# IST-DASLab/torch_cgx

Hardware: AMD Instinct MI355X
Metric: DDP samples/sec ResNet-50 4-bit (higher is better)
Workload: dtype bf16; 1 GPU; model=resnet50, global_batch=256, input=3x224x224, parallelism=dp1, backend=cgx, bits=4, bucket_size=1024, compression_active=False

## Files before the change

csrc/bindings.cc:

```cpp
#include <torch/extension.h>

#include <ATen/hip/impl/HIPStreamMasqueradingAsCUDA.h>
#include <torch/csrc/utils/pybind.h>

#include <ATen/hip/impl/HIPGuardImplMasqueradingAsCUDA.h>

#include <cstring>
#include <functional>
#include <thread>
#include <tuple>

#include "backend.h"
#include "bn_plan.h"
#include "collectives.h"
#include "conv1x1_plan.h"
#include "reducer.h"

namespace cgx {
namespace {

void run_rank_threads(int ws, int dev,
                      const std::function<void(int, hipStream_t)>& body,
                      const std::function<void()>& abort) {
  std::vector<hipStream_t> qs(ws, nullptr);
// ... 908 lines not shown
  }
  return out;
}

at::Tensor py_conv1x1_walk(int64_t rows, int64_t k, int64_t n,
                           int64_t max_workgroups) {
  const Conv1x1Plan p = conv1x1_plan(rows, k, n, (int)max_workgroups);
  TORCH_CHECK(p.eligible, "conv1x1_walk: shape is not eligible");
  return conv1x1_walk_of(p);
}


int clamp_workgroups(int64_t max_workgroups) {
  return (int)std::min<int64_t>(max_workgroups, 1 << 20);
}

bool py_conv1x1_bwd_eligible(const at::Tensor& dy, const at::Tensor& weight,
                             const c10::optional<at::Tensor>& skip) {
  if (!(bn_tensor_ok(dy) && weight.is_cuda() &&
        weight.device() == dy.device() &&
        weight.scalar_type() == at::kBFloat16 && weight.dim() == 4 &&
        weight.size(0) == dy.size(1) && weight.size(2) == 1 &&
        weight.size(3) == 1 && weight.is_contiguous() &&
        reinterpret_cast<uintptr_t>(weight.data_ptr()) % 16 == 0 &&
        conv1x1_bwd_plan(dy.numel() / dy.size(1), weight.size(1),
                         weight.size(0), skip.has_value())
            .eligible))
    return false;
  if (!skip.has_value()) return true;
  const at::Tensor& s = *skip;
  return s.dim() == 4 && s.size(0) == dy.size(0) &&
         s.size(1) == weight.size(1) && s.size(2) == dy.size(2) &&
         s.size(3) == dy.size(3) && s.device() == dy.device() &&
         bn_tensor_ok(s);
}

at::Tensor py_conv1x1_bwd_data(const at::Tensor& dy, const at::Tensor& weight,
                               const c10::optional<at::Tensor>& skip,
                               int64_t max_workgroups) {
  TORCH_CHECK(max_workgroups >= 0, "conv1x1_bwd_data: max_workgroups >= 0");
  TORCH_CHECK(py_conv1x1_bwd_eligible(dy, weight, skip),
              "conv1x1_bwd_data: dy, weight or skip is not eligible");
  const Conv1x1Plan p = conv1x1_bwd_plan(
      dy.numel() / dy.size(1), weight.size(1), weight.size(0),
      skip.has_value(), clamp_workgroups(max_workgroups));
  c10::hip::HIPGuardMasqueradingAsCUDA guard(dy.device().index());
  auto dx = at::empty({dy.size(0), p.n, dy.size(2), dy.size(3)}, dy.options(),
                      at::MemoryFormat::ChannelsLast);
  launch_conv1x1_bwd_data(p, dy.data_ptr(), weight.data_ptr(),
                          skip.has_value() ? skip->data_ptr() : nullptr,
                          dx.data_ptr(), bn_stream(dy));
  return dx;
}

py::dict py_conv1x1_bwd_plan(int64_t rows, int64_t k, int64_t n, bool with_add,
                             int64_t max_workgroups) {
  const Conv1x1Plan p =
      conv1x1_bwd_plan(rows, k, n, with_add, clamp_workgroups(max_workgroups));
  py::dict d;
  d["eligible"] = p.eligible;
  d["native"] = p.native;
  d["threads"] = kConvThreads;
  d["tile_rows"] = kConvTileRows;
  d["mfma_tiles"] = p.nt;
  d["tile_channels"] = p.bn;
  d["ntiles"] = p.ntiles;
  d["k_chunk"] = p.kc;
  d["k_chunks"] = p.nchunks;
  d["resident"] = p.resident;
  d["row_tiles"] = p.row_tiles;
  d["splits"] = p.splits;
  d["grid"] = p.grid;
  d["tiles_per_split"] = p.tiles_per_split;
  d["lds_bytes"] = p.lds_bytes;
  return d;
}

at::Tensor py_conv1x1_bwd_walk(int64_t rows, int64_t k, int64_t n,
                               bool with_add, int64_t max_workgroups) {
  const Conv1x1Plan p =
      conv1x1_bwd_plan(rows, k, n, with_add, clamp_workgroups(max_workgroups));
  TORCH_CHECK(p.eligible, "conv1x1_bwd_walk: shape is not eligible");
  return conv1x1_walk_of(p);
}

void py_register_layer(int64_t bucket_idx, int64_t layer_idx, int64_t numel,
                       int64_t bits, int64_t bucket_size) {
  Registry::get().register_layer((int)bucket_idx, (int)layer_idx, numel,
                                 (int)bits, (int)bucket_size);
}

void py_set_bits(int64_t bucket_idx, int64_t layer_idx, int64_t bits) {
  Registry::get().set_bits((int)bucket_idx, (int)layer_idx, (int)bits);
}

void py_set_bucket(int64_t bucket_idx, int64_t layer_idx,
                   int64_t bucket_size) {
  Registry::get().set_bucket_size((int)bucket_idx, (int)layer_idx,
                                  (int)bucket_size);
}

}
}

PYBIND11_MODULE(TORCH_EXTENSION_NAME, m) {
  py::class_<cgx::ProcessGroupCGX,
             c10::intrusive_ptr<cgx::ProcessGroupCGX>, c10d::Backend>(
      m, "ProcessGroupCGX")
      .def(py::init<c10::intrusive_ptr<c10d::Store>, int, int,
                    c10::intrusive_ptr<c10d::Backend>>(),
           py::arg("store"), py::arg("rank"), py::arg("size"),
           py::arg("cpu_delegate") = nullptr);

  m.def("register_layer", &cgx::py_register_layer, py::arg("bucket_idx"),
        py::arg("layer_idx"), py::arg("layer_numel"), py::arg("bits"),
        py::arg("bucket_size"));
  m.def("set_quantization_bits", &cgx::py_set_bits);
  m.def("set_quantization_bucket_size", &cgx::py_set_bucket);
  m.def("clear_registry", [] { cgx::Registry::get().clear(); });
  m.def("registry_match",
        [](int64_t numel, int64_t key) {
          cgx::Registry::BucketInfo info;
          const bool ok = cgx::Registry::get().next(
              numel, reinterpret_cast<const void*>(key), &info);
          return py::make_tuple(ok, ok ? info.idx : -1);
        },
        py::arg("numel"), py::arg("key") = 0);
  m.def("registry_snapshot", [] {
    py::list out;
    auto& reg = cgx::Registry::get();
    for (const auto& b : reg.snapshot()) {
      py::list numels, cfgs;
      for (auto n : b.numels) numels.append(n);
      for (const auto& c : b.cfgs)
        cfgs.append(py::make_tuple(c.bits, c.bucket_size));
      out.append(py::make_tuple(b.idx, numels, cfgs));
    }
    return out;
  });

  m.def("parse_engine_config", [] {
    auto c = cgx::EngineConfig::from_env();
    py::dict d;
    d["fusion_bytes"] = c.fusion_bytes;
    d["min_elems"] = c.min_elems;
    d["default_bits"] = c.default_bits;
    d["default_bucket"] = c.default_bucket;
    d["stochastic"] = c.stochastic;
    d["inner_ring"] = c.ring;
    d["cross_ring"] = c.cross_ring;
    d["debug_a2a"] = c.debug_a2a;
    d["fake_ratio"] = c.fake_ratio;
    d["skip_incomplete"] = c.skip_incomplete;
    d["dummy"] = c.dummy;
    d["intra_compress"] = c.intra_compress;
    d["intra_broadcast"] = c.intra_broadcast;
    d["error_feedback"] = c.error_feedback;
    return d;
  });
  m.def("env_flag", &cgx::env_flag, py::arg("name"),
        py::arg("default") = false,
        "Test seam: the textual boolean parser (only \"0\" is false).");
  m.def("env_int", &cgx::env_int, py::arg("name"), py::arg("default"),
        "Test seam: the numeric parser behind the `!= 0` booleans.");
  m.def("loopback_allreduce", &cgx::py_loopback_allreduce, py::arg("buckets"),
        "Run Reducer::allreduce (flat) at world_size=len(buckets) on one GPU "
// ... 51 lines not shown
        py::arg("dummy") = false,
        "Test seam: the bucket plan for layers laid out back to back from "
        "byte offset 0 -> (uncomp [(byte_off, count)], chunks [[(byte_off, "
        "numel, bits, bucket)]]).");
  m.def("plan_chunk", &cgx::py_plan_chunk, py::arg("views"), py::arg("dtype"),
        py::arg("ws"), py::arg("skip_incomplete") = false,
        "Test seam: the rank plan of one chunk [(byte_off, numel, bits, "
        "bucket)] -> (offs, szs, comp, rs [[(byte_off, n, bits, bucket, "
        "comp_off, skip_incomplete, fb_off)]]).");
  m.def("route_quantize", &cgx::py_route_quantize, py::arg("slices"),
        "Test seam: the launch router's quantize plan for "
        "[(in, out, fb, n, bits, bucket, skip_incomplete)] (pointers as "
        "ints) -> [(bits, kind, descs, cum, any_residual, max_gpl)].");
  m.def("route_dequantize", &cgx::py_route_dequantize, py::arg("slices"),
        py::arg("dtype"), py::arg("src_stride") = 0, py::arg("nsrc") = 1,
        py::arg("add") = false,
        "Test seam: the launch router's dequantize plan for "
        "[(in, out, n, bits, bucket, skip_incomplete)] -> "
        "[(bits, kind, descs, total_groups, any_residual)].");
  m.def("bn_act_forward", &cgx::py_bn_act_forward, py::arg("x"),
        py::arg("identity"), py::arg("weight"), py::arg("bias"),
        py::arg("running_mean"), py::arg("running_var"), py::arg("momentum"),
        py::arg("eps"), py::arg("relu"), py::arg("part") = py::none(),
        "Training-mode BatchNorm2d of a channels_last bf16 tensor, fused with "
        "an optional residual add and ReLU -> (out, mean, invstd, mask | "
        "None); updates the running statistics in place.  With `part`, the "
        "partials conv1x1_stats returned with x, the statistics pass over x "
        "is skipped.");
  m.def("bn_act_backward", &cgx::py_bn_act_backward, py::arg("dy"),
        py::arg("x"), py::arg("mean"), py::arg("invstd"), py::arg("weight"),
        py::arg("mask"), py::arg("has_identity"),
        "Backward of bn_act_forward -> (dx, dgamma, dbeta, didentity | None).");
  m.def("bn_act2_forward", &cgx::py_bn_act2_forward, py::arg("x3"),
        py::arg("xd"), py::arg("weight3"), py::arg("bias3"),
        py::arg("running_mean3"), py::arg("running_var3"),
        py::arg("momentum3"), py::arg("eps3"), py::arg("weightd"),
        py::arg("biasd"), py::arg("running_meand"), py::arg("running_vard"),
        py::arg("momentumd"), py::arg("epsd"), py::arg("relu"),
        py::arg("part3") = py::none(), py::arg("partd") = py::none(),
        "relu(bn3(x3) + bn_d(xd)) with both BatchNorms in training mode: "
        "(x3, xd, weight3, bias3, running_mean3, running_var3, momentum3, "
        "eps3, weightd, biasd, running_meand, running_vard, momentumd, epsd, "
        "relu, part3=None, partd=None) -> (out, mean3, invstd3, meand, "
        "invstdd, mask | None); part3 / partd as `part` of bn_act_forward.");
  m.def("conv1x1_stats", &cgx::py_conv1x1_stats, py::arg("x"),
        py::arg("weight"), py::arg("max_workgroups") = 0,
        "conv2d(x, weight) of a 1x1 / stride 1 / no-bias convolution on a "
        "channels_last bf16 tensor -> (y, part); part holds the per-channel "
        "(count, mean, M2) partials of y.  max_workgroups > 0 caps the "
        "persistent grid.");
  m.def("conv1x1_eligible", &cgx::py_conv1x1_eligible, py::arg("x"),
        py::arg("weight"),
        "True where conv1x1_stats takes (x, weight): CUDA, bf16, dense "
        "channels_last input, [N, K, 1, 1] weight, and a shape conv1x1_plan "
        "calls eligible.");
  m.def("conv1x1_plan", &cgx::py_conv1x1_plan, py::arg("rows"), py::arg("k"),
        py::arg("n"), py::arg("max_workgroups") = 0,
        "The launch geometry of conv1x1_stats for [rows, k] x [n, k], and "
        "`native`: whether the model uses it at this shape.");
  m.def("conv1x1_walk", &cgx::py_conv1x1_walk, py::arg("rows"), py::arg("k"),
        py::arg("n"), py::arg("max_workgroups") = 0,
        "Test seam: [grid, tiles_per_split, 4] int64, (row0, row1, n0, n1) "
        "of every tile each workgroup visits (-1: none).");
  m.def("conv1x1_bwd_data", &cgx::py_conv1x1_bwd_data, py::arg("dy"),
        py::arg("weight"), py::arg("skip") = py::none(),
        py::arg("max_workgroups") = 0,
        "Input gradient of conv2d(x, weight) for a 1x1 / stride 1 convolution "
        "on channels_last bf16 tensors, plus `skip` (a bf16 channels_last "
        "tensor of dx's shape) where given: dx = bf16(dy * W + skip), rounded "
        "once.  `skip` is not written.");
  m.def("conv1x1_bwd_eligible", &cgx::py_conv1x1_bwd_eligible, py::arg("dy"),
        py::arg("weight"), py::arg("skip") = py::none(),
        "True where conv1x1_bwd_data takes (dy, weight, skip).");
  m.def("conv1x1_bwd_plan", &cgx::py_conv1x1_bwd_plan, py::arg("rows"),
        py::arg("k"), py::arg("n"), py::arg("with_add") = false,
        py::arg("max_workgroups") = 0,
        "The launch geometry of conv1x1_bwd_data for dx [rows, k] from dy "
        "[rows, n], and `native`: whether the model uses it for this problem.");
  m.def("conv1x1_bwd_walk", &cgx::py_conv1x1_bwd_walk, py::arg("rows"),
        py::arg("k"), py::arg("n"), py::arg("with_add") = false,
        py::arg("max_workgroups") = 0,
        "Test seam: conv1x1_walk for the plan of conv1x1_bwd_plan; channels "
        "are dx's.");
  m.def("bn_act2_backward", &cgx::py_bn_act2_backward,
        "Backward of bn_act2_forward: (dy, x3, xd, mean3, invstd3, weight3, "
        "meand, invstdd, weightd, mask) -> (dx3, dxd, dgamma3, dbeta3, "
        "dgammad, dbetad).");
  m.def("bn_act_pool_forward", &cgx::py_bn_act_pool_forward, py::arg("x"),
        py::arg("weight"), py::arg("bias"), py::arg("running_mean"),
        py::arg("running_var"), py::arg("momentum"), py::arg("eps"),
        "max_pool2d(relu(bn(x)), 3, 2, 1) in training mode -> (pooled, mean, "
        "invstd, arg); arg is one byte per pooled element.");
  m.def("bn_act_pool_backward", &cgx::py_bn_act_pool_backward, py::arg("dy"),
        py::arg("x"), py::arg("mean"), py::arg("invstd"), py::arg("weight"),
        py::arg("arg"),
        "Backward of bn_act_pool_forward -> (dx, dgamma, dbeta).");
  m.def("bn_pool_geometry", &cgx::py_bn_pool_geometry, py::arg("h"),
        py::arg("w"),
        "Test seam: (windows [oh*ow, 9], covers [h*w, 4, 2]) of the stem's "
        "3x3/2/1 pooling as the kernels index it.");
  m.def("bn_eligible", &cgx::py_bn_eligible, py::arg("x"),
        "True where the fused BatchNorm kernels take `x`: CUDA, bf16, dense "
        "channels_last, and a shape bn_plan calls eligible.");
  m.def("bn_plan", &cgx::py_bn_plan, py::arg("rows"), py::arg("channels"),
        "Test seam: the launch geometry of the fused BatchNorm kernels for a "
        "[rows, channels] activation.");
  m.def("bn_sweep_indices", &cgx::py_bn_sweep_indices, py::arg("rows"),
        py::arg("channels"),
        "Test seam: [grid*threads, rows_per_thread+1] int64, the 16-byte "
        "vector indices every thread visits (-1: none).");
  m.def("bn_partial_offsets", &cgx::py_bn_partial_offsets, py::arg("rows"),
        py::arg("channels"), py::arg("wg"),
        "Test seam: the partial-buffer floats workgroup `wg` writes.");
  m.attr("FLAG_SKIP_INCOMPLETE") = cgx::kFlagSkipIncomplete;
  m.attr("FLAG_TAIL_ONLY") = cgx::kFlagTailOnly;
  m.attr("KIND_FAST") = (int)cgx::kFast;
  m.attr("KIND_GENERIC") = (int)cgx::kGeneric;
  m.attr("KIND_TWO_PASS") = (int)cgx::kTwoPass;
  m.attr("KIND_SUB") = (int)cgx::kSub;
}
```

csrc/conv1x1_kernels.hip:

```cpp
#include <hip/hip_runtime.h>

#include "bn_moments.h"
#include "check.h"
#include "conv1x1_plan.h"

namespace cgx {
namespace {

constexpr int kT = kConvThreads;

typedef __bf16 bf16x8 __attribute__((ext_vector_type(8)));
typedef __bf16 bf16x2 __attribute__((ext_vector_type(2)));
typedef float f32x2 __attribute__((ext_vector_type(2)));
typedef float f32x16 __attribute__((ext_vector_type(16)));

template <int KC>
__device__ inline int w_slot(int n, int q) {
  return n * (KC / 8) + (q ^ (KC == 64 ? (n >> 1) & 7 : n & 15));
}

__device__ inline int acc_row(int i, int h) {
  return (i & 3) + 8 * (i >> 2) + 4 * h;
}

// ... 288 lines not shown

#pragma unroll
    for (int jp = 0; jp < NT / 2; jp++) {
      uint4 sk[4];
      if (ADD) {
#pragma unroll
        for (int u = 0; u < 4; u++) {
          const int idx = u * 64 + lane, row = idx >> 3, q = idx & 7;
          sk[u] = make_uint4(0, 0, 0, 0);
          if (row < live)
            sk[u] = skip[(r0 + row) * nvec + (n0 + jp * 64) / 8 + q];
        }
      }
#pragma unroll
      for (int jj = 0; jj < 2; jj++)
#pragma unroll
        for (int e = 0; e < 16; e++) {
          const int row = acc_row(e, h);
          stagef[row * 64 + ((jj * 32 + c) ^ ((row & 1) << 2))] =
              acc[2 * jp + jj][e];
        }
      asm volatile("" ::: "memory");
      __builtin_amdgcn_wave_barrier();
#pragma unroll
      for (int u = 0; u < 4; u++) {
        const int idx = u * 64 + lane, row = idx >> 3, q = idx & 7;
        const uint4 lo = stage[row * 16 + 2 * q + (row & 1)];
        const uint4 hi = stage[row * 16 + 2 * q + ((row & 1) ^ 1)];
        float f[8] = {__uint_as_float(lo.x), __uint_as_float(lo.y),
                      __uint_as_float(lo.z), __uint_as_float(lo.w),
                      __uint_as_float(hi.x), __uint_as_float(hi.y),
                      __uint_as_float(hi.z), __uint_as_float(hi.w)};
        if (ADD) {
          const unsigned s4[4] = {sk[u].x, sk[u].y, sk[u].z, sk[u].w};
#pragma unroll
          for (int m = 0; m < 4; m++) {
            f[2 * m] += __uint_as_float(s4[m] << 16);
            f[2 * m + 1] += __uint_as_float(s4[m] & 0xffff0000u);
          }
        }
        const uint4 v = make_uint4(pack_bf16(f[0], f[1]), pack_bf16(f[2], f[3]),
                                   pack_bf16(f[4], f[5]), pack_bf16(f[6], f[7]));
        if (row < live) dx[(r0 + row) * nvec + (n0 + jp * 64) / 8 + q] = v;
      }
      asm volatile("" ::: "memory");
      __builtin_amdgcn_wave_barrier();
    }
  }
}

template <int NT, int KC, bool RES, bool ADD>
void launch_bwd(const Conv1x1Plan& p, const void* dy, const void* w,
                const void* skip, void* dx, hipStream_t stream) {
  static const hipError_t attr = hipFuncSetAttribute(
      reinterpret_cast<const void*>(&conv1x1_bwd_data<NT, KC, RES, ADD>),
      hipFuncAttributeMaxDynamicSharedMemorySize,
      kConvWLdsBytes + kConvBwdStageBytes);
  CGX_HIP_CHECK(attr);
  hipLaunchKernelGGL((conv1x1_bwd_data<NT, KC, RES, ADD>), dim3(p.grid),
                     dim3(kT), p.lds_bytes, stream,
                     static_cast<const uint4*>(dy),
                     static_cast<const uint4*>(w),
                     static_cast<const uint4*>(skip), static_cast<uint4*>(dx),
                     p);
}

template <int NT, bool ADD>
void launch_bwd_nt(const Conv1x1Plan& p, const void* dy, const void* w,
                   const void* skip, void* dx, hipStream_t stream) {
  if (p.kc == 64) launch_bwd<NT, 64, true, ADD>(p, dy, w, skip, dx, stream);
  else if (p.resident)
    launch_bwd<NT, 128, true, ADD>(p, dy, w, skip, dx, stream);
  else launch_bwd<NT, 128, false, ADD>(p, dy, w, skip, dx, stream);
}

template <bool ADD>
void launch_bwd_add(const Conv1x1Plan& p, const void* dy, const void* w,
                    const void* skip, void* dx, hipStream_t stream) {
  if (p.nt == 2) launch_bwd_nt<2, ADD>(p, dy, w, skip, dx, stream);
  else if (p.nt == 4) launch_bwd_nt<4, ADD>(p, dy, w, skip, dx, stream);
  else launch_bwd_nt<8, ADD>(p, dy, w, skip, dx, stream);
}

}

void launch_conv1x1_bwd_data(const Conv1x1Plan& p, const void* dy,
                             const void* w, const void* skip, void* dx,
                             hipStream_t stream) {
  TORCH_CHECK(p.eligible, "conv1x1_bwd_data: shape is not eligible");
  if (skip) launch_bwd_add<true>(p, dy, w, skip, dx, stream);
  else launch_bwd_add<false>(p, dy, w, skip, dx, stream);
  CGX_HIP_CHECK(hipGetLastError());
}

void launch_conv1x1_stats(const Conv1x1Plan& p, const void* x, const void* w,
                          void* y, float* part, hipStream_t stream) {
  TORCH_CHECK(p.eligible, "conv1x1_stats: shape is not eligible");
  if (p.nt == 2) launch_nt<2>(p, x, w, y, part, stream);
  else if (p.nt == 4) launch_nt<4>(p, x, w, y, part, stream);
  else launch_nt<8>(p, x, w, y, part, stream);
  CGX_HIP_CHECK(hipGetLastError());
}

}
```

csrc/conv1x1_plan.cc:

```cpp
#include "conv1x1_plan.h"

#include <algorithm>

namespace cgx {
namespace {

struct Measured {
  int k, n;
  int64_t rows;
};
constexpr Measured kNative[] = {
    {64, 64, 802816},   {64, 256, 802816},  {256, 64, 802816},
    {256, 128, 802816}, {128, 512, 200704}, {512, 128, 200704},
    {256, 1024, 50176},
};

bool measured_faster(int64_t rows, int k, int n) {
  for (const Measured& m : kNative)
    if (m.k == k && m.n == n && m.rows == rows) return true;
  return false;
}

bool pow2_in(int64_t v, int64_t lo, int64_t hi) {
  return v >= lo && v <= hi && (v & (v - 1)) == 0;
}

struct MeasuredBwd {
  int k, n;
  int64_t rows;
  bool with_add;
};
constexpr MeasuredBwd kNativeBwd[] = {
    {64, 64, 802816, true},    {256, 64, 802816, true},
    {256, 128, 802816, true},  {512, 128, 200704, true},
    {512, 256, 200704, true},  {1024, 256, 50176, true},
    {64, 256, 802816, false},  {128, 512, 200704, false},
};

bool measured_faster_bwd(int64_t rows, int k, int n, bool with_add) {
  for (const MeasuredBwd& m : kNativeBwd)
    if (m.k == k && m.n == n && m.rows == rows && m.with_add == with_add)
      return true;
  return false;
}

void tile_geometry(Conv1x1Plan& p, int stage_bytes) {
  p.nt = std::min(p.n / 32, kConvMaxNt);
  p.bn = 32 * p.nt;
  p.ntiles = p.n / p.bn;
  p.kc = p.k == 64 ? 64 : 128;
  p.nchunks = p.k / p.kc;
  p.resident = p.bn * p.k * 2 <= kConvWLdsBytes;
  p.lds_bytes = p.bn * (p.resident ? p.k : p.kc) * 2 + stage_bytes;
  p.row_tiles = (int)((p.rows + kConvTileRows - 1) / kConvTileRows);
}

int64_t splits_by_occupancy(const Conv1x1Plan& p, int by_regs) {
  const int per_cu = std::max(1, std::min(kConvLdsBytes / p.lds_bytes, by_regs));
  return std::min<int64_t>(p.row_tiles,
                           std::max(1, kConvCus * per_cu / p.ntiles));
}

void set_grid(Conv1x1Plan& p, int64_t splits, int max_workgroups) {
  if (max_workgroups > 0)
    splits = std::min<int64_t>(splits, std::max(1, max_workgroups / p.ntiles));
  p.splits = (int)splits;
  p.grid = p.ntiles * p.splits;
  p.tiles_per_split = (p.row_tiles + p.splits - 1) / p.splits;
}

}

Conv1x1Plan conv1x1_plan(int64_t rows, int64_t k, int64_t n,
                         int max_workgroups) {
  Conv1x1Plan p;
  p.rows = rows;
  p.eligible = pow2_in(k, 64, 2048) && pow2_in(n, 64, 2048) && rows >= 2 &&
               rows <= kBnMaxRows;
  if (!p.eligible) return p;
  p.k = (int)k;
  p.n = (int)n;
  p.native = measured_faster(rows, p.k, p.n);
  tile_geometry(p, kConvStageBytes);
  const int by_regs = p.nt == 8 ? 1 : p.nt == 4 ? 2 : 3;
  set_grid(p,
           std::min(splits_by_occupancy(p, by_regs),
                    std::max<int64_t>(1, rows / 82)),
           max_workgroups);
  p.run = 16 * p.tiles_per_split;
  p.pstride = 2 * p.n + p.ntiles;
  p.partial_floats = (int64_t)p.splits * p.pstride;
  return p;
}

Conv1x1Plan conv1x1_bwd_plan(int64_t rows, int64_t k, int64_t n, bool with_add,
                             int max_workgroups) {
  Conv1x1Plan p;
  p.rows = rows;
  p.eligible = pow2_in(k, 64, 2048) && pow2_in(n, 64, 2048) && rows >= 2 &&
               rows <= kBnMaxRows;
  if (!p.eligible) return p;
  p.k = (int)n;
  p.n = (int)k;
  p.native = measured_faster_bwd(rows, (int)k, (int)n, with_add);
  tile_geometry(p, kConvBwdStageBytes);
  const int by_regs = p.resident ? (p.nt == 8 ? 2 : p.nt == 4 ? 3 : 4)
                                 : (p.nt == 8 ? 1 : 2);
  set_grid(p, splits_by_occupancy(p, by_regs), max_workgroups);
  return p;
}

}
```

csrc/conv1x1_plan.h:

```cpp
#pragma once

#include <cstdint>

#include "bn_plan.h"

namespace cgx {

constexpr int kConvThreads = 256;
constexpr int kConvTileRows = 128;
constexpr int kConvMaxNt = 8;
constexpr int kConvCus = 256;
constexpr int kConvLdsBytes = 160 * 1024;
constexpr int kConvWLdsBytes = 128 * 1024;
constexpr int kConvStageBytes = 16 * 1024;
constexpr int kConvBwdStageBytes = 32 * 1024;

struct Conv1x1Plan {
  int64_t rows = 0;
  int k = 0, n = 0;
  bool eligible = false;
  bool native = false;
  int nt = 0;
  int bn = 0;
  int ntiles = 0;
  int kc = 0;
  int nchunks = 0;
  bool resident = false;
  int row_tiles = 0;
  int splits = 0;
  int grid = 0;
  int tiles_per_split = 0;
  int run = 0;
  int lds_bytes = 0;
  int pstride = 0;
  int64_t partial_floats = 0;
};

Conv1x1Plan conv1x1_plan(int64_t rows, int64_t k, int64_t n,
                         int max_workgroups = 0);

Conv1x1Plan conv1x1_bwd_plan(int64_t rows, int64_t k, int64_t n, bool with_add,
                             int max_workgroups = 0);

__host__ __device__ inline int conv1x1_ntile(const Conv1x1Plan& p, int wg) {
  return wg % p.ntiles;
}
__host__ __device__ inline int conv1x1_split(const Conv1x1Plan& p, int wg) {
  return wg / p.ntiles;
}
__host__ __device__ inline int conv1x1_tile(const Conv1x1Plan& p, int split,
                                            int i) {
  return split + i * p.splits;
}

inline BnPartials conv1x1_partials(const float* part, int n, int splits,
                                   int ntiles) {
  BnPartials q;
  q.mean = part;
  q.m2 = part + n;
  q.cnt = part + 2 * n;
  q.channels = n;
  q.splits = splits;
  q.tc = n / ntiles / 8;
  q.pstride = q.cstride = 2 * n + ntiles;
  return q;
}

void launch_conv1x1_stats(const Conv1x1Plan& p, const void* x, const void* w,
                          void* y, float* part, hipStream_t stream);

void launch_conv1x1_bwd_data(const Conv1x1Plan& p, const void* dy,
                             const void* w, const void* skip, void* dx,
                             hipStream_t stream);

}
```

torch_cgx_amd/ops/fused_bn.py:

```python

from __future__ import annotations

import os

import torch
import torch.nn.functional as F

from .. import _C


class _BnAct(torch.autograd.Function):
    @staticmethod
    def forward(ctx, x, identity, weight, bias, running_mean, running_var,
                momentum, eps, relu, part):
        out, mean, invstd, mask = _C.bn_act_forward(
            x, identity, weight, bias, running_mean, running_var, momentum,
            eps, relu, part)
        ctx.save_for_backward(x, mean, invstd, weight, mask)
        ctx.has_identity = identity is not None
        return out

    @staticmethod
    def backward(ctx, dy):
        x, mean, invstd, weight, mask = ctx.saved_tensors
# ... 26 lines not shown
                dbetad, None, None, None, None, None, None, None)


class _BnActPool(torch.autograd.Function):
    @staticmethod
    def forward(ctx, x, weight, bias, running_mean, running_var, momentum,
                eps):
        out, mean, invstd, arg = _C.bn_act_pool_forward(
            x, weight, bias, running_mean, running_var, momentum, eps)
        ctx.save_for_backward(x, mean, invstd, weight, arg)
        return out

    @staticmethod
    def backward(ctx, dy):
        x, mean, invstd, weight, arg = ctx.saved_tensors
        dx, dgamma, dbeta = _C.bn_act_pool_backward(dy, x, mean, invstd,
                                                    weight, arg)
        return (dx, dgamma, dbeta, None, None, None, None)


def fused_bn_enabled() -> bool:
    return os.environ.get("CGX_FUSED_BN", "1") != "0"


def _native(bn, x, identity) -> bool:
    if not (bn.training and bn.track_running_stats
            and bn.momentum is not None and fused_bn_enabled()):
        return False
    if bn.weight is None or bn.bias is None:
        return False
    if not (x.is_cuda and _C.bn_eligible(x)):
        return False
    if identity is not None and not (
            identity.shape == x.shape and identity.device == x.device
            and _C.bn_eligible(identity)):
        return False
    return bn.weight.dtype == torch.float32


def _bn_args(bn):
    return (bn.weight, bn.bias, bn.running_mean, bn.running_var, bn.momentum,
            bn.eps)


def bn_act(bn: torch.nn.BatchNorm2d, x: torch.Tensor,
           identity: torch.Tensor = None, relu: bool = True,
           identity_bn: torch.nn.BatchNorm2d = None,
           part: torch.Tensor = None,
           identity_part: torch.Tensor = None) -> torch.Tensor:
    if identity_bn is not None:
        if _native(bn, x, identity) and _native(identity_bn, identity, x):
            bn.num_batches_tracked.add_(1)
            identity_bn.num_batches_tracked.add_(1)
            return _BnActJoin.apply(x, identity, *_bn_args(bn),
                                    *_bn_args(identity_bn), relu, part,
                                    identity_part)
        out = bn(x) + identity_bn(identity)
        return F.relu(out, inplace=True) if relu else out
    if _native(bn, x, identity):
        bn.num_batches_tracked.add_(1)
        return _BnAct.apply(x, identity, *_bn_args(bn), relu, part)
    out = bn(x)
    if identity is not None:
        out = out + identity
    if relu:
        out = F.relu(out, inplace=True)
    return out


class _Conv1x1Stats(torch.autograd.Function):

    @staticmethod
    @torch.amp.custom_fwd(device_type="cuda", cast_inputs=torch.bfloat16)
    def forward(ctx, x, weight):
        y, part = _C.conv1x1_stats(x, weight)
        ctx.save_for_backward(x, weight)
        ctx.mark_non_differentiable(part)
        return y, part

    @staticmethod
    @torch.amp.custom_bwd(device_type="cuda")
    def backward(ctx, dy, _dpart):
        x, weight = ctx.saved_tensors
        dx, dw, _ = torch.ops.aten.convolution_backward(
            dy, x, weight, None, (1, 1), (0, 0), (1, 1), False, (0, 0), 1,
            (ctx.needs_input_grad[0], ctx.needs_input_grad[1], False))
        return dx, dw


class _Conv1x1Fork(torch.autograd.Function):

    @staticmethod
    @torch.amp.custom_fwd(device_type="cuda", cast_inputs=torch.bfloat16)
    def forward(ctx, x, weight, native_fwd, fork):
        if native_fwd:
            y, part = _C.conv1x1_stats(x, weight)
            ctx.mark_non_differentiable(part)
        else:
            y, part = F.conv2d(x, weight), None
        ctx.save_for_backward(x, weight)
        ctx.set_materialize_grads(False)
        return y, part, (x.view_as(x) if fork else None)

    @staticmethod
    @torch.amp.custom_bwd(device_type="cuda")
    def backward(ctx, dy, _dpart, dskip):
        x, weight = ctx.saved_tensors
        dx = dw = None
        if dy is not None and ctx.needs_input_grad[1]:
            dw = _conv1x1_backward(dy, x, weight, (False, True, False))[1]
        if ctx.needs_input_grad[0]:
            dx = dskip if dy is None else _conv1x1_dx(dy, x, weight, dskip)
        return dx, dw, None, None


def _conv1x1_backward(dy, x, weight, mask):
    return torch.ops.aten.convolution_backward(
        dy, x, weight, None, (1, 1), (0, 0), (1, 1), False, (0, 0), 1, mask)


def _conv1x1_dx(dy, x, weight, dskip):
    mode = native_conv1x1_bwd_mode()
    if mode != "0" and _C.conv1x1_bwd_eligible(dy, weight, dskip):
        plan = _C.conv1x1_bwd_plan(x.numel() // x.shape[1], x.shape[1],
                                   weight.shape[0], dskip is not None)
        if plan["native"] or mode == "all":
            return _C.conv1x1_bwd_data(dy, weight, dskip)
    dx = _conv1x1_backward(dy, x, weight, (True, False, False))[0]
    return dx if dskip is None else dx + dskip


def native_conv1x1_mode() -> str:
    if not fused_bn_enabled():
        return "0"
    return os.environ.get("CGX_NATIVE_CONV1X1", "1")


def native_conv1x1_bwd_mode() -> str:
    if native_conv1x1_mode() == "0":
        return "0"
    return os.environ.get("CGX_NATIVE_CONV1X1_BWD", "1")


def _conv1x1_shape(conv, bn, x):
    if native_conv1x1_mode() == "0":
        return None
    if not (type(conv) is torch.nn.Conv2d and conv.kernel_size == (1, 1)
            and conv.stride == (1, 1) and conv.padding == (0, 0)
            and conv.dilation == (1, 1) and conv.groups == 1
            and conv.bias is None and conv.padding_mode == "zeros"):
        return None
    if not (bn.training and bn.track_running_stats
            and bn.momentum is not None and bn.weight is not None
            and bn.bias is not None and bn.weight.dtype == torch.float32):
        return None
    if not (x.is_cuda and x.dim() == 4 and x.dtype == torch.bfloat16
            and _C.bn_eligible(x)):
        return None
    w = conv.weight
    autocast = (torch.is_autocast_enabled("cuda")
                and torch.get_autocast_dtype("cuda") == torch.bfloat16)
    if not (w.device == x.device and w.shape[1] == x.shape[1]
            and (w.dtype == torch.bfloat16
                 or (autocast and w.dtype == torch.float32))):
        return None
    if w.dtype == torch.bfloat16 and not _C.conv1x1_eligible(x, w):
        return None
    return x.numel() // x.shape[1], x.shape[1], w.shape[0]


def _conv1x1_native(shape) -> bool:
    plan = _C.conv1x1_plan(*shape)
    return plan["eligible"] and (plan["native"]
                                 or native_conv1x1_mode() == "all")


def _conv1x1_bwd_native(shape, with_add) -> bool:
    mode = native_conv1x1_bwd_mode()
    if mode == "0":
        return False
    plan = _C.conv1x1_bwd_plan(*shape, with_add)
    return plan["eligible"] and (plan["native"] or mode == "all")


def _conv(conv, bn, x, fork=False):
    shape = _conv1x1_shape(conv, bn, x)
    if shape is None:
        return conv(x), None, x
    fwd = _conv1x1_native(shape)
    if torch.is_grad_enabled():
        fork = fork and _conv1x1_bwd_native(shape, True)
        if fork or _conv1x1_bwd_native(shape, False):
            y, part, skip = _Conv1x1Fork.apply(x, conv.weight, fwd, fork)
            return y, part, (skip if fork else x)
    if fwd:
        return _Conv1x1Stats.apply(x, conv.weight) + (x,)
    return conv(x), None, x


def conv_bn_act(conv: torch.nn.Conv2d, bn: torch.nn.BatchNorm2d,
                x: torch.Tensor, identity: torch.Tensor = None,
                relu: bool = True, identity_conv: torch.nn.Conv2d = None,
                identity_bn: torch.nn.BatchNorm2d = None) -> torch.Tensor:
    y, part, _ = _conv(conv, bn, x)
    if identity_conv is None:
        return bn_act(bn, y, identity, relu, part=part)
    yd, partd, _ = _conv(identity_conv, identity_bn, identity)
    return bn_act(bn, y, yd, relu, identity_bn=identity_bn, part=part,
                  identity_part=partd)


def conv_bn_act_fork(conv: torch.nn.Conv2d, bn: torch.nn.BatchNorm2d,
                     x: torch.Tensor, relu: bool = True):
    y, part, skip = _conv(conv, bn, x, fork=True)
    return bn_act(bn, y, None, relu, part=part), skip


def _pool_is_3x3_s2_p1(pool) -> bool:
    def pair(v):
        return tuple(v) if isinstance(v, (tuple, list)) else (v, v)

    return (type(pool) is torch.nn.MaxPool2d
            and pair(pool.kernel_size) == (3, 3) and pair(pool.stride) == (2, 2)
            and pair(pool.padding) == (1, 1) and pair(pool.dilation) == (1, 1)
            and not pool.ceil_mode and not pool.return_indices)


def bn_act_pool(bn: torch.nn.BatchNorm2d, x: torch.Tensor,
                pool: torch.nn.Module) -> torch.Tensor:
    if _pool_is_3x3_s2_p1(pool) and _native(bn, x, None):
        bn.num_batches_tracked.add_(1)
        return _BnActPool.apply(x, *_bn_args(bn))
    return pool(bn_act(bn, x))
```

Measured before the change: 7967 samples/s.

## Add native MFMA split-K weight-gradient kernel for 1x1 convolutions

Adds a HIP kernel that computes the weight gradient of 1x1 stride-1 convolutions as dy^T·x with bf16 MFMA. Rows are split across workgroups, each workgroup writes an fp32 partial, and a separate finalize kernel reduces the partials and rounds once to bf16. The kernel uses LDS transpose reads and register double-buffered loads. It replaces the aten convolution_backward weight path for a measured list of ResNet-50 shapes, which aims to cut the cost of library wrw kernels. In exchange it adds a partial-sum buffer, a second launch, and a split dx/dw call on some paths.

```diff
diff --git a/csrc/bindings.cc b/csrc/bindings.cc
--- a/csrc/bindings.cc
+++ b/csrc/bindings.cc
@@ -1014,6 +1014,78 @@
       conv1x1_bwd_plan(rows, k, n, with_add, clamp_workgroups(max_workgroups));
   TORCH_CHECK(p.eligible, "conv1x1_bwd_walk: shape is not eligible");
   return conv1x1_walk_of(p);
+}
+
+
+bool py_conv1x1_wrw_eligible(const at::Tensor& dy, const at::Tensor& x) {
+  return bn_tensor_ok(dy) && bn_tensor_ok(x) && x.device() == dy.device() &&
+         x.size(0) == dy.size(0) && x.size(2) == dy.size(2) &&
+         x.size(3) == dy.size(3) &&
+         conv1x1_wrw_plan(dy.numel() / dy.size(1), x.size(1), dy.size(1))
+             .eligible;
+}
+
+at::Tensor py_conv1x1_wrw(const at::Tensor& dy, const at::Tensor& x,
+                          int64_t max_workgroups) {
+  TORCH_CHECK(max_workgroups >= 0, "conv1x1_wrw: max_workgroups >= 0");
+  TORCH_CHECK(py_conv1x1_wrw_eligible(dy, x),
+              "conv1x1_wrw: dy or x is not eligible");
+  const Conv1x1WrwPlan p =
+      conv1x1_wrw_plan(dy.numel() / dy.size(1), x.size(1), dy.size(1),
+                       clamp_workgroups(max_workgroups));
+  c10::hip::HIPGuardMasqueradingAsCUDA guard(dy.device().index());
+  auto dw = at::empty({p.n, p.k, 1, 1}, dy.options(),
+                      at::MemoryFormat::ChannelsLast);
+  auto part = at::empty({p.splits, p.n, p.k}, dy.options().dtype(at::kFloat));
+  launch_conv1x1_wrw(p, dy.data_ptr(), x.data_ptr(), part.data_ptr<float>(),
+                     dw.data_ptr(), bn_stream(dy));
+  return dw;
+}
+
+py::dict py_conv1x1_wrw_plan(int64_t rows, int64_t k, int64_t n,
+                             int64_t max_workgroups) {
+  const Conv1x1WrwPlan p =
+      conv1x1_wrw_plan(rows, k, n, clamp_workgroups(max_workgroups));
+  py::dict d;
+  d["eligible"] = p.eligible;
+  d["native"] = p.native;
+  d["threads"] = kConvThreads;
+  d["bn"] = p.bn;
+  d["bk"] = p.bk;
+  d["ntiles_n"] = p.ntiles_n;
+  d["ntiles_k"] = p.ntiles_k;
+  d["chunk_rows"] = p.chunk_rows;
+  d["row_chunks"] = p.row_chunks;
+  d["splits"] = p.splits;
+  d["grid"] = p.grid;
+  d["chunks_per_split"] = p.chunks_per_split;
+  d["lds_bytes"] = p.lds_bytes;
+  d["partial_floats"] = p.partial_floats;
+  return d;
+}
+
+at::Tensor py_conv1x1_wrw_walk(int64_t rows, int64_t k, int64_t n,
+                               int64_t max_workgroups) {
+  const Conv1x1WrwPlan p =
+      conv1x1_wrw_plan(rows, k, n, clamp_workgroups(max_workgroups));
+  TORCH_CHECK(p.eligible, "conv1x1_wrw_walk: shape is not eligible");
+  auto out = at::full({p.grid, p.chunks_per_split, 5}, -1,
+                      at::TensorOptions().dtype(at::kLong));
+  int64_t* o = out.data_ptr<int64_t>();
+  for (int wg = 0; wg < p.grid; wg++) {
+    const int tile = conv1x1_wrw_tile(p, wg), split = conv1x1_wrw_split(p, wg);
+    for (int i = 0; i < p.chunks_per_split; i++) {
+      const int ch = conv1x1_wrw_chunk(p, split, i);
+      if (ch >= p.row_chunks) break;
+      int64_t* e = o + ((int64_t)wg * p.chunks_per_split + i) * 5;
+      e[0] = (int64_t)(tile / p.ntiles_k) * p.bn;
+      e[1] = (int64_t)(tile % p.ntiles_k) * p.bk;
+      e[2] = split;
+      e[3] = (int64_t)ch * p.chunk_rows;
+      e[4] = std::min<int64_t>(e[3] + p.chunk_rows, p.rows);
+    }
+  }
+  return out;
 }
 
 void py_register_layer(int64_t bucket_idx, int64_t layer_idx, int64_t numel,
@@ -1231,6 +1303,23 @@
         py::arg("max_workgroups") = 0,
         "Test seam: conv1x1_walk for the plan of conv1x1_bwd_plan; channels "
         "are dx's.");
+  m.def("conv1x1_wrw", &cgx::py_conv1x1_wrw, py::arg("dy"), py::arg("x"),
+        py::arg("max_workgroups") = 0,
+        "Weight gradient of conv2d(x, weight) for a 1x1 / stride 1 convolution "
+        "on channels_last bf16 tensors: dw[n, k] = bf16(sum_r dy[r, n] * "
+        "x[r, k]) as [N, K, 1, 1], accumulated in fp32 in a fixed order and "
+        "rounded once.");
+  m.def("conv1x1_wrw_eligible", &cgx::py_conv1x1_wrw_eligible, py::arg("dy"),
+        py::arg("x"), "True where conv1x1_wrw takes (dy, x).");
+  m.def("conv1x1_wrw_plan", &cgx::py_conv1x1_wrw_plan, py::arg("rows"),
+        py::arg("k"), py::arg("n"), py::arg("max_workgroups") = 0,
+        "The launch geometry of conv1x1_wrw for dw [n, k] from dy [rows, n] "
+        "and x [rows, k], and `native`: whether the model uses it for this "
+        "problem.");
+  m.def("conv1x1_wrw_walk", &cgx::py_conv1x1_wrw_walk, py::arg("rows"),
+        py::arg("k"), py::arg("n"), py::arg("max_workgroups") = 0,
+        "Test seam: [grid, chunks_per_split, 5] int64, (n0, k0, split, row0, "
+        "row1) of every row chunk each workgroup visits (-1: none).");
   m.def("bn_act2_backward", &cgx::py_bn_act2_backward,
         "Backward of bn_act2_forward: (dy, x3, xd, mean3, invstd3, weight3, "
         "meand, invstdd, weightd, mask) -> (dx3, dxd, dgamma3, dbeta3, "
diff --git a/csrc/conv1x1_kernels.hip b/csrc/conv1x1_kernels.hip
--- a/csrc/conv1x1_kernels.hip
+++ b/csrc/conv1x1_kernels.hip
@@ -394,6 +394,185 @@
   else launch_bwd_nt<8, ADD>(p, dy, w, skip, dx, stream);
 }
 
+
+typedef __bf16 bf16x4 __attribute__((ext_vector_type(4)));
+typedef __attribute__((address_space(3))) bf16x4 lds_bf16x4;
+
+template <int C>
+__device__ inline int wrw_cell(int r, int u) {
+  const int lin = r * (C / 32) + u;
+  const int swz = C == 64 ? (r >> 1) & 1 : r & 3;
+  return 256 * (lin >> 2) + 64 * ((lin & 3) ^ swz);
+}
+
+template <int C>
+__device__ inline void wrw_load(uint4 (&v)[C / 32], const uint4* __restrict__ src,
+                                int width, int c0, int64_t r0, int64_t rows,
+                                int tid) {
+#pragma unroll
+  for (int i = 0; i < C / 32; i++) {
+    const int idx = tid + i * kT, row = idx / (C / 8), q = idx % (C / 8);
+    const bool live = r0 + row < rows;
+    const int64_t r = live ? r0 + row : rows - 1;
+    const uint4 t = src[(r * width + c0) / 8 + q];
+    v[i] = live ? t : make_uint4(0, 0, 0, 0);
+  }
+}
+
+template <int C>
+__device__ inline void wrw_store(char* img, const uint4 (&v)[C / 32], int tid) {
+#pragma unroll
+  for (int i = 0; i < C / 32; i++) {
+    const int idx = tid + i * kT, row = idx / (C / 8), q = idx % (C / 8);
+    *reinterpret_cast<uint4*>(img + wrw_cell<C>(row, q >> 2) + 16 * (q & 3)) =
+        v[i];
+  }
+}
+
+template <int C>
+__device__ inline bf16x8 wrw_operand(char* img, int base, int s) {
+  char* a = img + base + s * 16 * 2 * C;
+  const bf16x4 lo = __builtin_amdgcn_ds_read_tr16_b64_v4bf16(
+      (lds_bf16x4*)a);
+  const bf16x4 hi = __builtin_amdgcn_ds_read_tr16_b64_v4bf16(
+      (lds_bf16x4*)(a + 4 * 2 * C));
+  return __builtin_shufflevector(lo, hi, 0, 1, 2, 3, 4, 5, 6, 7);
+}
+
+template <int BN, int BK>
+__global__ __launch_bounds__(kT) void conv1x1_wrw(
+    const uint4* __restrict__ dy, const uint4* __restrict__ x,
+    float* __restrict__ part, Conv1x1WrwPlan p) {
+  extern __shared__ uint4 lds[];
+  constexpr int MT = BN / 64, KT = BK / 64;
+  char* img_n = reinterpret_cast<char*>(lds);
+  char* img_k = img_n + kWrwChunkRows * BN * 2;
+  const int tid = threadIdx.x, wave = tid >> 6, lane = tid & 63;
+  const int c = lane & 31, h = lane >> 5;
+  const int wn = wave >> 1, wk = wave & 1;
+  const int tile = conv1x1_wrw_tile(p, blockIdx.x);
+  const int split = conv1x1_wrw_split(p, blockIdx.x);
+  const int n0 = (tile / p.ntiles_k) * BN, k0 = (tile % p.ntiles_k) * BK;
+
+  const int q = (lane >> 2) & 3;
+  const int in_cell = 32 * ((lane >> 4) & 1) + 8 * (lane & 3);
+  int an[MT], ak[KT];
+#pragma unroll
+  for (int j = 0; j < MT; j++)
+    an[j] = wrw_cell<BN>(8 * h + q, wn * MT + j) + in_cell;
+#pragma unroll
+  for (int j = 0; j < KT; j++)
+    ak[j] = wrw_cell<BK>(8 * h + q, wk * KT + j) + in_cell;
+
+  f32x16 acc[MT][KT];
+#pragma unroll
+  for (int jm = 0; jm < MT; jm++)
+#pragma unroll
+    for (int jk = 0; jk < KT; jk++)
+#pragma unroll
+      for (int e = 0; e < 16; e++) acc[jm][jk][e] = 0.f;
+
+  uint4 vn[BN / 32], vk[BK / 32];
+  wrw_load<BN>(vn, dy, p.n, n0, (int64_t)split * kWrwChunkRows, p.rows, tid);
+  wrw_load<BK>(vk, x, p.k, k0, (int64_t)split * kWrwChunkRows, p.rows, tid);
+
+  for (int i = 0; i < p.chunks_per_split; i++) {
+    if (conv1x1_wrw_chunk(p, split, i) >= p.row_chunks) break;
+    __syncthreads();
+    wrw_store<BN>(img_n, vn, tid);
+    wrw_store<BK>(img_k, vk, tid);
+    __syncthreads();
+    const int next = conv1x1_wrw_chunk(p, split, i + 1);
+    if (next < p.row_chunks) {
+      wrw_load<BN>(vn, dy, p.n, n0, (int64_t)next * kWrwChunkRows, p.rows, tid);
+      wrw_load<BK>(vk, x, p.k, k0, (int64_t)next * kWrwChunkRows, p.rows, tid);
+    }
+#pragma unroll
+    for (int s = 0; s < kWrwChunkRows / 16; s++) {
+      bf16x8 a[MT], b[KT];
+#pragma unroll
+      for (int j = 0; j < MT; j++) a[j] = wrw_operand<BN>(img_n, an[j], s);
+#pragma unroll
+      for (int j = 0; j < KT; j++) b[j] = wrw_operand<BK>(img_k, ak[j], s);
+#pragma unroll
+      for (int jm = 0; jm < MT; jm++)
+#pragma unroll
+        for (int jk = 0; jk < KT; jk++)
+          acc[jm][jk] = __builtin_amdgcn_mfma_f32_32x32x16_bf16(
+              a[jm], b[jk], acc[jm][jk], 0, 0, 0);
+    }
+  }
+
+  float* out = part + (int64_t)split * p.n * p.k;
+#pragma unroll
+  for (int jm = 0; jm < MT; jm++)
+#pragma unroll
+    for (int jk = 0; jk < KT; jk++)
+#pragma unroll
+      for (int e = 0; e < 16; e++) {
+        const int n = n0 + (wn * MT + jm) * 32 + acc_row(e, h);
+        const int k = k0 + (wk * KT + jk) * 32 + c;
+        out[(int64_t)n * p.k + k] = acc[jm][jk][e];
+      }
+}
+
+__global__ __launch_bounds__(kT) void conv1x1_wrw_finalize(
+    const float4* __restrict__ part, uint4* __restrict__ dw, int splits,
+    int64_t vecs, int g) {
+  const int lane = threadIdx.x & 63, vw = 64 / g;
+  const int64_t wave = ((int64_t)blockIdx.x * kT + threadIdx.x) >> 6;
+  const int64_t v = wave * vw + lane % vw;
+  const int j = lane / vw, per = (splits + g - 1) / g;
+  const int s1 = (j + 1) * per < splits ? (j + 1) * per : splits;
+  float f[8] = {0.f, 0.f, 0.f, 0.f, 0.f, 0.f, 0.f, 0.f};
+  for (int s = j * per; s < s1; s++) {
+    const float4 lo = part[(s * vecs + v) * 2];
+    const float4 hi = part[(s * vecs + v) * 2 + 1];
+    f[0] += lo.x, f[1] += lo.y, f[2] += lo.z, f[3] += lo.w;
+    f[4] += hi.x, f[5] += hi.y, f[6] += hi.z, f[7] += hi.w;
+  }
+  for (int off = 32; off >= vw; off >>= 1)
+#pragma unroll
+    for (int e = 0; e < 8; e++) f[e] += __shfl_down(f[e], off);
+  if (j == 0)
+    dw[v] = make_uint4(pack_bf16(f[0], f[1]), pack_bf16(f[2], f[3]),
+                       pack_bf16(f[4], f[5]), pack_bf16(f[6], f[7]));
+}
+
+template <int BN, int BK>
+void launch_wrw(const Conv1x1WrwPlan& p, const void* dy, const void* x,
+                float* part, hipStream_t stream) {
+  hipLaunchKernelGGL((conv1x1_wrw<BN, BK>), dim3(p.grid), dim3(kT),
+                     p.lds_bytes, stream, static_cast<const uint4*>(dy),
+                     static_cast<const uint4*>(x), part, p);
+}
+
+template <int BN>
+void launch_wrw_bn(const Conv1x1WrwPlan& p, const void* dy, const void* x,
+                   float* part, hipStream_t stream) {
+  if (p.bk == 64) launch_wrw<BN, 64>(p, dy, x, part, stream);
+  else if (p.bk == 128) launch_wrw<BN, 128>(p, dy, x, part, stream);
+  else if constexpr (BN < 256) launch_wrw<BN, 256>(p, dy, x, part, stream);
+  else TORCH_CHECK(false, "conv1x1_wrw: no 256 x 256 tile");
+}
+
+}
+
+void launch_conv1x1_wrw(const Conv1x1WrwPlan& p, const void* dy, const void* x,
+                        float* part, void* dw, hipStream_t stream) {
+  TORCH_CHECK(p.eligible, "conv1x1_wrw: shape is not eligible");
+  if (p.bn == 64) launch_wrw_bn<64>(p, dy, x, part, stream);
+  else if (p.bn == 128) launch_wrw_bn<128>(p, dy, x, part, stream);
+  else launch_wrw_bn<256>(p, dy, x, part, stream);
+  CGX_HIP_CHECK(hipGetLastError());
+  const int64_t vecs = (int64_t)p.n * p.k / 8;
+  int g = 1;
+  while (g < 16 && 2 * g <= p.splits && vecs * g < 4 * kConvCus * kT) g *= 2;
+  hipLaunchKernelGGL(conv1x1_wrw_finalize, dim3((unsigned)(vecs * g / kT)),
+                     dim3(kT), 0, stream,
+                     reinterpret_cast<const float4*>(part),
+                     static_cast<uint4*>(dw), p.splits, vecs, g);
+  CGX_HIP_CHECK(hipGetLastError());
 }
 
 void launch_conv1x1_bwd_data(const Conv1x1Plan& p, const void* dy,
diff --git a/csrc/conv1x1_plan.cc b/csrc/conv1x1_plan.cc
--- a/csrc/conv1x1_plan.cc
+++ b/csrc/conv1x1_plan.cc
@@ -69,6 +69,59 @@
   p.tiles_per_split = (p.row_tiles + p.splits - 1) / p.splits;
 }
 
+constexpr Measured kNativeWrw[] = {
+    {64, 256, 802816},  {256, 64, 802816},  {256, 128, 802816},
+    {128, 512, 200704}, {512, 128, 200704}, {512, 256, 200704},
+    {256, 1024, 50176}, {1024, 256, 50176}, {1024, 512, 50176},
+    {512, 2048, 12544}, {2048, 512, 12544},
+};
+
+bool measured_faster_wrw(int64_t rows, int k, int n) {
+  for (const Measured& m : kNativeWrw)
+    if (m.k == k && m.n == n && m.rows == rows) return true;
+  return false;
+}
+
+}
+
+Conv1x1WrwPlan conv1x1_wrw_plan(int64_t rows, int64_t k, int64_t n,
+                                int max_workgroups) {
+  Conv1x1WrwPlan p;
+  p.rows = rows;
+  p.eligible = pow2_in(k, 64, 2048) && pow2_in(n, 64, 2048) && rows >= 2 &&
+               rows <= kBnMaxRows;
+  if (!p.eligible) return p;
+  p.k = (int)k;
+  p.n = (int)n;
+  p.native = measured_faster_wrw(rows, p.k, p.n);
+  p.chunk_rows = kWrwChunkRows;
+  p.row_chunks = (int)((rows + kWrwChunkRows - 1) / kWrwChunkRows);
+  const int64_t cap = std::min<int64_t>(
+      p.row_chunks, std::max<int64_t>(1, rows * (n + k) / (8 * n * k)));
+  p.bn = (int)std::min<int64_t>(n, 256);
+  p.bk = (int)std::min<int64_t>(k, 256);
+  if (p.bn == 256 && p.bk == 256) p.bn = 128;
+  while (cap < p.row_chunks && std::max(p.bn, p.bk) > 128 &&
+         (n / p.bn) * (k / p.bk) * cap < kConvCus)
+    (p.bn >= p.bk ? p.bn : p.bk) /= 2;
+  p.ntiles_n = p.n / p.bn;
+  p.ntiles_k = p.k / p.bk;
+  p.lds_bytes = kWrwChunkRows * (p.bn + p.bk) * 2;
+  const int acc_tiles = (p.bn / 64) * (p.bk / 64);
+  const int by_regs =
+      acc_tiles == 1 ? 4 : acc_tiles == 2 ? 3 : acc_tiles == 4 ? 2 : 1;
+  const int per_cu = std::min(kConvLdsBytes / p.lds_bytes, by_regs);
+  const int tiles = p.ntiles_n * p.ntiles_k;
+  int64_t splits =
+      std::min<int64_t>(cap, std::max(1, kConvCus * per_cu / tiles));
+  if (splits > 8) splits -= splits % 8;
+  if (max_workgroups > 0)
+    splits = std::min<int64_t>(splits, std::max(1, max_workgroups / tiles));
+  p.splits = (int)splits;
+  p.grid = tiles * p.splits;
+  p.chunks_per_split = (p.row_chunks + p.splits - 1) / p.splits;
+  p.partial_floats = (int64_t)p.splits * p.n * p.k;
+  return p;
 }
 
 Conv1x1Plan conv1x1_plan(int64_t rows, int64_t k, int64_t n,
diff --git a/csrc/conv1x1_plan.h b/csrc/conv1x1_plan.h
--- a/csrc/conv1x1_plan.h
+++ b/csrc/conv1x1_plan.h
@@ -66,6 +66,48 @@
   return q;
 }
 
+constexpr int kWrwChunkRows = 64;
+
+struct Conv1x1WrwPlan {
+  int64_t rows = 0;
+  int k = 0, n = 0;
+  bool eligible = false;
+  bool native = false;
+  int bn = 0, bk = 0;
+  int ntiles_n = 0, ntiles_k = 0;
+  int chunk_rows = 0;
+  int row_chunks = 0;
+  int splits = 0;
+  int grid = 0;
+  int chunks_per_split = 0;
+  int lds_bytes = 0;
+  int64_t partial_floats = 0;
+};
+
+Conv1x1WrwPlan conv1x1_wrw_plan(int64_t rows, int64_t k, int64_t n,
+                                int max_workgroups = 0);
+
+__host__ __device__ inline int conv1x1_wrw_tiles(const Conv1x1WrwPlan& p) {
+  return p.ntiles_n * p.ntiles_k;
+}
+__host__ __device__ inline int conv1x1_wrw_tile(const Conv1x1WrwPlan& p,
+                                                int wg) {
+  const int tiles = conv1x1_wrw_tiles(p);
+  return p.splits % 8 == 0 ? (wg / 8) % tiles : wg % tiles;
+}
+__host__ __device__ inline int conv1x1_wrw_split(const Conv1x1WrwPlan& p,
+                                                 int wg) {
+  const int tiles = conv1x1_wrw_tiles(p);
+  return p.splits % 8 == 0 ? (wg / 8 / tiles) * 8 + wg % 8 : wg / tiles;
+}
+__host__ __device__ inline int conv1x1_wrw_chunk(const Conv1x1WrwPlan& p,
+                                                 int split, int i) {
+  return split + i * p.splits;
+}
+
+void launch_conv1x1_wrw(const Conv1x1WrwPlan& p, const void* dy, const void* x,
+                        float* part, void* dw, hipStream_t stream);
+
 void launch_conv1x1_stats(const Conv1x1Plan& p, const void* x, const void* w,
                           void* y, float* part, hipStream_t stream);
 
diff --git a/torch_cgx_amd/ops/fused_bn.py b/torch_cgx_amd/ops/fused_bn.py
--- a/torch_cgx_amd/ops/fused_bn.py
+++ b/torch_cgx_amd/ops/fused_bn.py
@@ -132,9 +132,14 @@
     @torch.amp.custom_bwd(device_type="cuda")
     def backward(ctx, dy, _dpart):
         x, weight = ctx.saved_tensors
-        dx, dw, _ = torch.ops.aten.convolution_backward(
-            dy, x, weight, None, (1, 1), (0, 0), (1, 1), False, (0, 0), 1,
-            (ctx.needs_input_grad[0], ctx.needs_input_grad[1], False))
+        need_dx, need_dw = ctx.needs_input_grad[:2]
+        if need_dw and _conv1x1_dw_native(dy, x):
+            dw = _conv1x1_dw(dy, x, weight)
+            dx = None
+            if need_dx:
+                dx = _conv1x1_backward(dy, x, weight, (True, False, False))[0]
+            return dx, dw
+        dx, dw, _ = _conv1x1_backward(dy, x, weight, (need_dx, need_dw, False))
         return dx, dw
 
 
@@ -158,7 +163,7 @@
         x, weight = ctx.saved_tensors
         dx = dw = None
         if dy is not None and ctx.needs_input_grad[1]:
-            dw = _conv1x1_backward(dy, x, weight, (False, True, False))[1]
+            dw = _conv1x1_dw(dy, x, weight)
         if ctx.needs_input_grad[0]:
             dx = dskip if dy is None else _conv1x1_dx(dy, x, weight, dskip)
         return dx, dw, None, None
@@ -167,6 +172,21 @@
 def _conv1x1_backward(dy, x, weight, mask):
     return torch.ops.aten.convolution_backward(
         dy, x, weight, None, (1, 1), (0, 0), (1, 1), False, (0, 0), 1, mask)
+
+
+def _conv1x1_dw_native(dy, x) -> bool:
+    mode = native_conv1x1_wrw_mode()
+    if mode == "0" or not _C.conv1x1_wrw_eligible(dy, x):
+        return False
+    plan = _C.conv1x1_wrw_plan(x.numel() // x.shape[1], x.shape[1],
+                               dy.shape[1])
+    return plan["native"] or mode == "all"
+
+
+def _conv1x1_dw(dy, x, weight):
+    if _conv1x1_dw_native(dy, x):
+        return _C.conv1x1_wrw(dy, x)
+    return _conv1x1_backward(dy, x, weight, (False, True, False))[1]
 
 
 def _conv1x1_dx(dy, x, weight, dskip):
@@ -192,6 +212,12 @@
     return os.environ.get("CGX_NATIVE_CONV1X1_BWD", "1")
 
 
+def native_conv1x1_wrw_mode() -> str:
+    if native_conv1x1_mode() == "0":
+        return "0"
+    return os.environ.get("CGX_NATIVE_CONV1X1_WRW", "1")
+
+
 def _conv1x1_shape(conv, bn, x):
     if native_conv1x1_mode() == "0":
         return None
@@ -230,6 +256,14 @@
     if mode == "0":
         return False
     plan = _C.conv1x1_bwd_plan(*shape, with_add)
+    return plan["eligible"] and (plan["native"] or mode == "all")
+
+
+def _conv1x1_wrw_native(shape) -> bool:
+    mode = native_conv1x1_wrw_mode()
+    if mode == "0":
+        return False
+    plan = _C.conv1x1_wrw_plan(*shape)
     return plan["eligible"] and (plan["native"] or mode == "all")
 
 
@@ -240,7 +274,8 @@
     fwd = _conv1x1_native(shape)
     if torch.is_grad_enabled():
         fork = fork and _conv1x1_bwd_native(shape, True)
-        if fork or _conv1x1_bwd_native(shape, False):
+        if (fork or _conv1x1_bwd_native(shape, False)
+                or _conv1x1_wrw_native(shape)):
             y, part, skip = _Conv1x1Fork.apply(x, conv.weight, fwd, fork)
             return y, part, (skip if fork else x)
     if fwd:
```

After: 8237 samples/s (median of 6 runs). +3.4%, better.
